# ucla-rlcourse/competitive-rl

Measured on AMD Instinct MI355X. Metric: env-steps/sec (whole node), cPongDouble 65536 envs per GPU, higher is better.
Workload: dtype u8; 1 GPU; cPongDouble-v0 raw (N,2,210,160,3) u8, 1 step = 1 frame (BASELINE config #2); envs_per_gpu=65536, gather=n/a, actions=uniform random, pre-generated on device, auto_reset=True

## Files before the change

### competitive_rl_amd/_native.py

```python
import ctypes as C
import os

import numpy as np

PKG = os.path.dirname(os.path.abspath(__file__))
LIB_PATH = os.path.join(PKG, "libcrl_hip_%s.so" % os.environ["CRL_LIB_VARIANT"] if os.environ.get("CRL_LIB_VARIANT") else "libcrl_hip.so")

CRL_ENV_PONG_DOUBLE, CRL_ENV_CAR_DOUBLE, CRL_ENV_PONG_SINGLE, CRL_ENV_CAR_SINGLE = 1, 2, 3, 4
CRL_FLAG_STACK_REPLICATE = 1
CAR_MAX_TILES = 512
CAR_MAP_ORG, CAR_MAP_W = 4392, 1216
CRL_OBS_RAW_RGB, CRL_OBS_GRAY_RESIZED = 0, 1
PONG_FRAME_BYTES = 210 * 160 * 3
ATLAS_BYTES = 22 * 22 * 34 * 160

CRL_LEAGUE_MAX_AGENTS = 16
CRL_LEAGUE_RANDOM, CRL_LEAGUE_RULE_BASED, CRL_LEAGUE_LIGHT = 0, 1, 2
CRL_POOL_KIND_FULL = 3
CRL_LEAGUE_DOMAIN_OPPONENT, CRL_LEAGUE_DOMAIN_ACTION, CRL_LEAGUE_DOMAIN_SAMPLE = 0x4C47554F, 0x4C475541, 0x4C475553
CRL_LEDGER_DOMAIN_OPPONENT = 0x4C475557
CRL_LEDGER_COUNTERS = 6
CRL_LEDGER_COUNTER_NAMES = ("episodes", "wins", "losses", "draws", "return_sum", "length_sum")
CRL_LEDGER_PFSP_HARD, CRL_LEDGER_PFSP_VARIANCE = 0, 1
CRL_ARENA_DOMAIN_PAIR = 0x4C475550
# ... 67 lines not shown
    "crl_car_get_track": (i32, [vp, i64, vp, vp, vp, vp, vp, vp]),
    "crl_car_set_track": (i32, [vp, i64, i32, vp, vp, vp, vp, vp]),
    "crl_car_get_map": (i32, [vp, i64, vp, vp, vp]),
    "crl_car_set_replay": (i32, [vp, vp, vp, i64]),
    "crl_policy_create": (i32, [i32, i64, vp, vp, vp, vp, vp, vp, P(vp)]),
    "crl_policy_create_full": (i32, [i32, i64, vp, vp, vp, vp, vp, vp, vp, vp, P(vp)]),
    "crl_policy_destroy": (None, [vp]),
    "crl_policy_reset": (i32, [vp, vp]),
    "crl_policy_act": (i32, [vp, vp, i64, vp, i64, vp, vp]),
    "crl_policy_get_stack": (i32, [vp, vp, vp]),
    "crl_policy_set_stack": (i32, [vp, vp, vp]),
    "crl_policy_set_sampling": (i32, [vp, f32, f32, u64, i64]),
    "crl_policy_set_critic": (i32, [vp, vp, vp]),
    "crl_policy_act_rollout": (i32, [vp, vp, i64, vp, vp, i64, vp, vp, vp, vp]),
    "crl_policy_load_weights": (i32, [vp, vp, vp, vp, vp, vp, vp, vp, vp, vp, vp, vp]),
    "crl_terminal_observation_dev": (i32, [vp, vp, i64, vp, vp]),
    "crl_check": (i32, [vp, vp]),
    "crl_car_info": (i32, [vp, P(vp), P(vp)]),
    "crl_car_copy_info": (i32, [vp, vp, vp, vp, vp]),
    "crl_frame_stack_update": (i32, [vp, vp, i32, i64, vp, i64, i32, i32, i64, vp]),
    "crl_frame_stack_update_to": (i32, [vp, vp, vp, i32, i64, vp, i64, i32, i32, i64, vp]),
    "crl_frame_stack_update_u8": (i32, [vp, vp, vp, i32, i64, vp, i64, i32, i32, i64, vp]),
    "crl_ctx_last_error": (cstr, [vp]),
    "crl_obs_descriptors": (i32, [vp, vp, vp]),
    "crl_render_frames_dev": (i32, [vp, vp, i64, vp, vp]),
    "crl_car_cap_hits": (i32, [vp, vp, vp]),
    "crl_selftest_sincosf": (i32, [i32, u64, u64, vp]),
    "crl_step_stack": (i32, [vp, vp, vp, vp, vp, P(CrlStackDesc), vp]),
    "crl_draw_stack": (i32, [vp, vp, P(CrlStackDesc), vp]),
    "crl_set_flags_event": (i32, [vp, vp]),
    "crl_kernel_time_stats": (i32, [vp, i32, P(f64), P(i64), P(f64)]),
    "crl_draw_raw_delta": (i32, [vp, vp, vp, i32, vp]),
    "crl_step_raw_delta": (i32, [vp, vp, vp, vp, vp, vp, vp]),
    "crl_league_create": (i32, [i32, i64, i64, u64, P(vp)]),
    "crl_league_destroy": (None, [vp]),
    "crl_league_add_builtin": (i32, [vp, i32]),
    "crl_league_add_light": (i32, [vp, vp, vp, vp, vp, vp, vp]),
    "crl_pool_add_full": (i32, [vp, vp, vp, vp, vp, vp, vp, vp, vp, i64]),
    "crl_pool_load_light": (i32, [vp, i32, vp, vp, vp, vp, vp, vp, vp]),
    "crl_pool_load_full": (i32, [vp, i32, vp, vp, vp, vp, vp, vp, vp, vp, vp]),
    "crl_sampling_set_agent": (i32, [vp, i32, f32, f32]),
    "crl_sampling_get_agent": (i32, [vp, i32, P(f32), P(f32)]),
    "crl_league_seed": (i32, [vp, u64, vp]),
    "crl_league_set_assignment": (i32, [vp, vp, i32, vp]),
    "crl_league_get_assignment": (i32, [vp, vp, vp]),
    "crl_league_resample": (i32, [vp, vp, vp]),
    "crl_league_get_lists": (i32, [vp, vp, vp, vp]),
    "crl_league_act": (i32, [vp, vp, i64, vp, i64, vp, vp]),
    "crl_league_reset": (i32, [vp, vp]),
    "crl_league_get_stack": (i32, [vp, vp, vp]),
    "crl_league_set_stack": (i32, [vp, vp, vp]),
    "crl_ledger_create": (i32, [i32, i64, i64, u64, i32, P(vp)]),
    "crl_ledger_destroy": (None, [vp]),
    "crl_ledger_seed": (i32, [vp, u64, vp]),
    "crl_ledger_reset": (i32, [vp, vp]),
    "crl_ledger_set_agents": (i32, [vp, i32, vp]),
    "crl_ledger_set_weights": (i32, [vp, vp, i32, vp]),
    "crl_ledger_get_weights": (i32, [vp, vp, vp]),
    "crl_ledger_pfsp_weights": (i32, [vp, vp, i32, i32, u32, vp]),
    "crl_ledger_get_counters": (i32, [vp, vp, vp, vp]),
    "crl_ledger_set_counters": (i32, [vp, vp, vp, vp]),
    "crl_ledger_get_env_state": (i32, [vp, vp, vp, vp, vp]),
    "crl_ledger_set_env_state": (i32, [vp, vp, vp, vp, vp]),
    "crl_ledger_step": (i32, [vp, vp, vp, i64, vp, i32, vp, vp]),
    "crl_arena_create": (i32, [i32, i64, i64, u64, i32, P(vp)]),
    "crl_arena_destroy": (None, [vp]),
# ... 71 lines not shown
```

### competitive_rl_amd/csrc/crl_api.hip

```cpp
#include <math.h>
#include <stdarg.h>
#include <stdio.h>
#include <string.h>

#include <algorithm>
#include <string>
#include <vector>

#include "crl_internal.h"
#include "pong_band_span.h"
#include "pong_device.h"

using namespace crl;

static thread_local std::string g_err;
static thread_local std::string *g_ctx_err = nullptr;

void crl_fail_no_ctx(void) { g_ctx_err = nullptr; }

int crl_fail(int code, const char *fmt, ...) {
    char buf[512];
    va_list ap;
    va_start(ap, fmt);
    vsnprintf(buf, sizeof(buf), fmt, ap);
// ... 7 lines not shown
    std::vector<int32_t> ofs, si;
    std::vector<float> alpha;
};

static AreaTab area_table(int ssize, int dsize) {
    AreaTab t;
    const double scale = 1.0 / ((double)dsize / (double)ssize);
    for (int d = 0; d < dsize; d++) {
        t.ofs.push_back((int32_t)t.si.size());
        const double f1 = d * scale, f2 = f1 + scale;
        const double cell = std::min(scale, ssize - f1);
        int s1 = (int)ceil(f1), s2 = (int)floor(f2);
        s2 = std::min(s2, ssize - 1);
        s1 = std::min(s1, s2);
        if (s1 - f1 > 1e-3) t.si.push_back(s1 - 1), t.alpha.push_back((float)((s1 - f1) / cell));
        for (int s = s1; s < s2; s++) t.si.push_back(s), t.alpha.push_back((float)(1.0 / cell));
        if (f2 - s2 > 1e-3) t.si.push_back(s2), t.alpha.push_back((float)(std::min(std::min(f2 - s2, 1.0), cell) / cell));
    }
    t.ofs.push_back((int32_t)t.si.size());
    return t;
}


struct crl_ctx {
    std::string err;
    crl_opts o;
    int64_t n;
    PongSoA s{};
    ServeSrc src{};
    std::vector<void *> allocs;
    uint8_t *atlas_rgb = nullptr;
    uint8_t *band_span = nullptr;
    int ink_row0 = 0, ink_row1 = 0;
    GrayTables gray{};
    uint8_t *tile_hdr = nullptr;
    double *ru = nullptr;
    uint8_t *rbx = nullptr, *rby = nullptr;
    crl_timer tm;
    uint64_t *gather = nullptr;
    int64_t gather_cap = 0;
    int64_t *idx_dev = nullptr;
    int64_t idx_cap = 0;
    int32_t *bad_action_host = nullptr, *bad_action_dev = nullptr;
    std::vector<uint8_t> atlas_host;
    hipEvent_t flags_ev = nullptr;
    crl_car_ctx *car = nullptr;
};

template <class T>
static int dev_alloc(crl_ctx *c, T **p, size_t count) {
    void *q = nullptr;
    HIP_TRY(hipMalloc(&q, std::max<size_t>(count * sizeof(T), 16)));
    c->allocs.push_back(q);
    *p = (T *)q;
    return CRL_OK;
}

template <class T>
static int dev_upload(crl_ctx *c, T **p, const std::vector<T> &v, size_t pad_to = 0) {
    size_t cnt = std::max(v.size(), pad_to);
    int rc = dev_alloc(c, p, cnt);
    if (rc) return rc;
    HIP_TRY(hipMemset(*p, 0, std::max<size_t>(cnt * sizeof(T), 16)));
    HIP_TRY(hipMemcpy(*p, v.data(), v.size() * sizeof(T), hipMemcpyHostToDevice));
    return CRL_OK;
}
// ... 231 lines not shown
        if (e == hipSuccess) e = hipMemset(c->s.num_steps, 0, n * 4);
        if (e == hipSuccess) e = hipMemset(c->s.real_reward, 0, n * 8);
        if (e == hipSuccess) e = hipMemcpy(c->s.keep, blank.data(), 2 * n * 8, hipMemcpyHostToDevice);
        if (e == hipSuccess) e = hipMemcpy(c->s.ring, blank.data(), 8 * n * 8, hipMemcpyHostToDevice);
        if (e == hipSuccess) e = hipMemcpy(c->s.obs_frames, blank.data(), 2 * n * 8, hipMemcpyHostToDevice);
        if (e == hipSuccess) e = hipMemcpy(c->s.term_frames, blank.data(), 2 * n * 8, hipMemcpyHostToDevice);
        if (e == hipSuccess) e = hipHostMalloc((void **)&c->bad_action_host, 64, hipHostMallocMapped);
        if (e == hipSuccess) {
            *c->bad_action_host = 0;
            e = hipHostGetDevicePointer((void **)&c->bad_action_dev, c->bad_action_host, 0);
        }
        if (e != hipSuccess) {
            crl_destroy(c);
            return crl_fail(CRL_EHIP, "create: state initialisation: %s", hipGetErrorString(e));
        }
        c->s.bad_action = c->bad_action_dev;
    }
    c->src.seed = opts->seed, c->src.env_id_base = opts->env_id_base;
    int r0 = CRL_PONG_TOP, r1 = 0;
    for (int sp = 0; sp < 484; sp++)
        for (int r = 0; r < CRL_PONG_TOP; r++)
            for (int x = 0; x < CRL_PONG_W; x++)
                if (c->atlas_host[((size_t)sp * CRL_PONG_TOP + r) * CRL_PONG_W + x] != 255) r0 = std::min(r0, r), r1 = std::max(r1, r + 1);
    if (r1 <= r0) r0 = r1 = 0;
    c->ink_row0 = r0, c->ink_row1 = r1;
    if (opts->obs_mode == CRL_OBS_RAW_RGB) {
        std::vector<uint8_t> rgb((size_t)CRL_PONG_ATLAS_BYTES * 3);
        for (size_t i = 0; i < (size_t)CRL_PONG_ATLAS_BYTES; i++) rgb[3 * i] = rgb[3 * i + 1] = rgb[3 * i + 2] = c->atlas_host[i];
        rc = dev_upload(c, &c->atlas_rgb, rgb);
        std::vector<uint8_t> span(pong_band_span_bytes(22));
        const int bad = pong_band_span_table(c->atlas_host.data(), 22, CRL_PONG_TOP, CRL_PONG_W, r0, r1, span.data());
        if (!rc && bad) rc = crl_fail(CRL_ESTATE, "score atlas: transition %d changes a pixel outside the ink rows [%d, %d)", bad - 1, r0, r1);
        if (!rc) rc = dev_upload(c, &c->band_span, span);
    } else {
        rc = setup_gray(c);
    }
    if (rc) { crl_destroy(c); return rc; }
    hipError_t e = hipDeviceSynchronize();
    if (e != hipSuccess) { crl_destroy(c); return crl_fail(CRL_EHIP, "create: %s", hipGetErrorString(e)); }
    *out = c;
    return CRL_OK;
}

void crl_destroy(crl_ctx *c) {
    g_ctx_err = nullptr;
    if (!c) return;
    hipSetDevice(c->o.device);
    hipDeviceSynchronize();
#ifdef CRL_ABLATION
    if (getenv("CRL_GRAY_DEBUG") && (atoi(getenv("CRL_GRAY_DEBUG")) & 128)) pong_gray_print_ticks();
#endif
    if (c->car) crl_car_destroy(c->car);
    for (void *p : c->allocs) hipFree(p);
    for (int w = 0; w < kTimerSlots; w++)
        for (auto &p : c->tm.ev[w]) hipEventDestroy(p.a), hipEventDestroy(p.b);
    for (auto &p : c->tm.pool) hipEventDestroy(p.a), hipEventDestroy(p.b);
    if (c->ru) hipFree(c->ru);
    if (c->rbx) hipFree(c->rbx);
    if (c->rby) hipFree(c->rby);
    if (c->gather) hipFree(c->gather);
    if (c->idx_dev) hipFree(c->idx_dev);
    if (c->bad_action_host) hipHostFree(c->bad_action_host);
    delete c;
}

int crl_seed(crl_ctx *c, uint64_t seed) {
// ... 129 lines not shown
    }
    end_timed(c, 1, st);
    HIP_TRY(hipGetLastError());
    return CRL_OK;
}

int crl_step_raw_delta(crl_ctx *c, const void *actions_void, uint8_t *obs_dev, uint64_t *drawn_dev, float *rew_dev, uint8_t *done_dev, void *stream) {
    CRL_ENTER(c);
    if (!c || !actions_void || !obs_dev || !drawn_dev) return crl_fail(CRL_EINVAL, "null argument");
    if (c->car || c->o.obs_mode != CRL_OBS_RAW_RGB) return crl_fail(CRL_ESTATE, "crl_step_raw_delta needs a Pong RAW_RGB context");
    if ((uintptr_t)obs_dev % 16) return crl_fail(CRL_EINVAL, "crl_step_raw_delta: obs_dev must be 16-byte aligned");
    if ((uintptr_t)drawn_dev % 8) return crl_fail(CRL_EINVAL, "crl_step_raw_delta: drawn_dev must be 8-byte aligned");
    if (int rc = pending_action_error(c, true)) return rc;
    hipStream_t st = (hipStream_t)stream;
    if (c->flags_ev) {
        begin_timed(c, 0, st);
        launch_pong_dynamics(c->s, c->src, (const int32_t *)actions_void, c->n, pong_mode(c), rew_dev, done_dev, st);
        end_timed(c, 0, st);
        HIP_TRY(hipGetLastError());
        HIP_TRY(hipEventRecord(c->flags_ev, st));
        begin_timed(c, 1, st);
        launch_pong_raster_raw_delta(c->s.obs_frames, drawn_dev, c->n, c->atlas_rgb, c->band_span, c->ink_row0, c->ink_row1, obs_dev, pong_views(c), st);
        end_timed(c, 1, st);
        HIP_TRY(hipGetLastError());
        return CRL_OK;
    }
#ifdef CRL_ABLATION
    if (getenv("CRL_RAW_STEP_SPLIT") && atoi(getenv("CRL_RAW_STEP_SPLIT"))) {
        begin_timed(c, 0, st);
        launch_pong_dynamics(c->s, c->src, (const int32_t *)actions_void, c->n, pong_mode(c), rew_dev, done_dev, st);
        end_timed(c, 0, st);
        begin_timed(c, 1, st);
        launch_pong_step_raw_delta(c->s, c->src, (const int32_t *)actions_void, c->n, rew_dev, done_dev, drawn_dev, c->atlas_rgb, c->band_span,
                                   c->ink_row0, c->ink_row1, obs_dev, pong_views(c), st, 1);
        end_timed(c, 1, st);
        HIP_TRY(hipGetLastError());
        return CRL_OK;
    }
#endif
    begin_timed(c, 1, st);
    launch_pong_step_raw_delta(c->s, c->src, (const int32_t *)actions_void, c->n, rew_dev, done_dev, drawn_dev, c->atlas_rgb, c->band_span, c->ink_row0,
                               c->ink_row1, obs_dev, pong_views(c), st);
    end_timed(c, 1, st);
    HIP_TRY(hipGetLastError());
    return CRL_OK;
}

int crl_set_flags_event(crl_ctx *c, void *event) {
    CRL_ENTER(c);
    if (!c) return crl_fail(CRL_EINVAL, "null ctx");
    if (c->car) return crl_fail(CRL_ESTATE, "crl_set_flags_event is a Pong entry point");
    c->flags_ev = (hipEvent_t)event;
    return CRL_OK;
}

int crl_draw_stack(crl_ctx *c, uint8_t *obs_dev, const crl_stack_desc *stack, void *stream) {
    CRL_ENTER(c);
    if (!c || !stack) return crl_fail(CRL_EINVAL, "null argument");
    GrayStack sk;
    if (int rc = stack_of(c, stack, &sk)) return rc;
    return draw_obs(c, obs_dev, (hipStream_t)stream, &sk);
}

int crl_info(crl_ctx *c, const float **real_reward_dev, const int32_t **num_steps_dev) {
    CRL_ENTER(c);
    if (!c) return crl_fail(CRL_EINVAL, "null ctx");
    if (c->car) return crl_fail(CRL_ESTATE, "crl_info is a Pong entry point");
    if (real_reward_dev) *real_reward_dev = c->s.real_reward;
    if (num_steps_dev) *num_steps_dev = c->s.num_steps;
    return CRL_OK;
}

int crl_copy_info(crl_ctx *c, float *rr_out, int32_t *ns_out, void *stream) {
    CRL_ENTER(c);
    if (!c) return crl_fail(CRL_EINVAL, "null ctx");
    if (c->car) return crl_fail(CRL_ESTATE, "crl_copy_info is a Pong entry point");
    hipStream_t st = (hipStream_t)stream;
// ... 325 lines not shown
```

### competitive_rl_amd/csrc/pong_device.h

```cpp
#pragma once
#include <hip/hip_runtime.h>
#include <stdint.h>

#include "../../include/crl.h"

namespace crl {

struct PongSoA {
    double *speed_x, *speed_y;
    int32_t *ball_x, *ball_y, *bat_l, *bat_r, *score_l, *score_r, *rounds, *steps, *wrap_steps;
    uint32_t *serve_ctr;
    uint64_t *keep;
    uint64_t *ring;
    uint64_t *obs_frames;
    uint64_t *term_frames;
    float *real_reward;
    int32_t *num_steps;
    int32_t *bad_action;
};

struct ServeSrc {
    uint64_t seed;
    int64_t env_id_base;
    const double *ru;
// ... 172 lines not shown
    if (!action_ok(a.x) || !action_ok(a.y)) *s.bad_action = (action_ok(a.x) ? a.y : a.x) + 1;
    int r_l, r_r;
    const bool done = frame_step(e, a.x, a.y, src, i, r_l, r_r);
    const float fl = (float)r_l, fr = (float)r_r;
    if (rew) {
        if (single) rew[i] = fl;
        else reinterpret_cast<float2 *>(rew)[i] = make_float2(fl, fr);
    }
    reinterpret_cast<float2 *>(s.real_reward)[i] = make_float2(fl, fr);
    if (done) {
        const uint64_t t = frame_of(e);
        s.term_frames[i] = t, s.term_frames[n + i] = t;
        game_reset(e, src, i);
    }
    if (done_out) done_out[i] = done ? 1 : 0;
    const uint64_t f = frame_of(e);
    s.obs_frames[i] = f;
    store_env(s, i, e);
    return f;
}

struct PongMode {
    bool wrapped, single, replicate;
};
void launch_pong_reset(const PongSoA &s, const ServeSrc &src, int64_t n, PongMode mode, hipStream_t st);
void launch_pong_dynamics(const PongSoA &s, const ServeSrc &src, const int32_t *actions, int64_t n, PongMode mode,
                          float *rew, uint8_t *done, hipStream_t st);
void launch_pong_gather_frames(const uint64_t *frames, const int64_t *idx_dev, int64_t count, int64_t n, uint64_t *ring_out,
                               hipStream_t st);
void launch_pong_raster_raw(const uint64_t *frames, int64_t n, const uint8_t *atlas_rgb, int ink_row0, int ink_row1,
                            uint8_t *obs, int views, hipStream_t st);
void launch_pong_raster_raw_delta(const uint64_t *frames, uint64_t *drawn, int64_t n, const uint8_t *atlas_rgb, const uint8_t *band_span,
                                  int ink_row0, int ink_row1, uint8_t *obs, int views, hipStream_t st);
void launch_pong_step_raw_delta(const PongSoA &s, const ServeSrc &src, const int32_t *actions, int64_t n, float *rew, uint8_t *done,
                                uint64_t *drawn, const uint8_t *atlas_rgb, const uint8_t *band_span, int ink_row0, int ink_row1, uint8_t *obs,
                                int views, hipStream_t st, int stepped = 0);

struct GrayTabOfs {
    int xa, ya, xs0, xn, ys0, yn, xf, xl, yf, yl, total, fast_ok, max_taps;
    int xa255, rowstatic, colstatic;
    int box32;
};
struct GrayStack {
    uint8_t *out;
    int k, view;
    int f32;
    int valid;
    int alias;
};
struct GrayTables {
    int R;
    uint8_t *atlas_gray;
    uint8_t *band;
    int band_rows, band_chunks;
    int32_t *xofs, *yofs;
    int32_t *xsi, *ysi;
    float *xalpha, *yalpha;
    uint8_t *rest;
    int zero_row0, zero_row1;
    uint8_t *x_first, *x_last;
    uint8_t *y_first, *y_last;
    uint8_t *tab_blob;
    GrayTabOfs tofs;
    float *f32_top;
    float *f32_bot;
    int f32_bot0;
    int f32_xtaps, f32_ytaps;
    int f32_map_row0, f32_map_rows;
};
// ... 16 lines not shown
```

### competitive_rl_amd/csrc/pong_raster_raw.hip

```cpp
#include <stdlib.h>

#include "crl_internal.h"
#include "pong_band_span.h"
#include "pong_device.h"

namespace crl {

static constexpr int kRowBytes = CRL_PONG_W * 3;
static constexpr int kRowChunks = kRowBytes / 16;
static constexpr int kFrameChunks = CRL_PONG_H * kRowChunks;

__device__ inline uint32_t nibble_to_bytes(uint32_t nib) {
    return ((nib * 0x00204081u) & 0x01010101u) * 0xFFu;
}

__device__ inline uint32_t span_bits(int a, int b) {
    a = max(a, 0), b = min(b, 16);
    return a < b ? (((1u << b) - 1u) & ~((1u << a) - 1u)) : 0u;
}

__device__ inline uint32_t bswap32(uint32_t v) { return __builtin_bswap32(v); }

__device__ __forceinline__ uint4 raw_chunk(const Frame &f, int q, const uint4 *__restrict__ atlas_rgb, int ink_row0, int ink_row1, int dbg) {
    const bool blank = f.sl == 255;
    const uint32_t bg = blank ? 0u : 0xFFFFFFFFu;
    const int view = q >= kFrameChunks;
    const int c = q - view * kFrameChunks;
    const int row = c / kRowChunks;
    const int cc = c - row * kRowChunks;
    const bool mirror = view && row >= CRL_PONG_MIRROR_ROW;
    const int sc = mirror ? (kRowChunks - 1 - cc) : cc;
    uint4 v = make_uint4(bg, bg, bg, bg);
    if (!blank && !(dbg & 1)) {
// ... 78 lines not shown

#endif

template <int ITERS, int VIEWS>
__global__ __launch_bounds__(256) void pong_raster_raw_sweep_kernel(const uint64_t *__restrict__ frames, const uint4 *__restrict__ atlas_rgb,
                                                                    int ink_row0, int ink_row1, uint4 *__restrict__ obs, int64_t n, int dbg) {
    constexpr int per_env = VIEWS * kFrameChunks;
    const int64_t total = n * per_env;
    const int64_t stride = (int64_t)gridDim.x * 256;
    Frame f0[ITERS], f1[ITERS];
    int q0[ITERS];
#pragma unroll
    for (int i = 0; i < ITERS; i++) {
        int64_t g0 = (int64_t)blockIdx.x * 256 + i * stride;
        g0 = g0 < total ? g0 : total - 1;
        const int64_t e0 = g0 / per_env;
        const int64_t e1 = e0 + 1 < n ? e0 + 1 : e0;
        f0[i] = unpack_frame(frames[e0]), f1[i] = unpack_frame(frames[e1]);
        q0[i] = (int)(g0 - e0 * per_env);
    }
#pragma unroll
    for (int i = 0; i < ITERS; i++) {
        const int64_t g = (int64_t)blockIdx.x * 256 + i * stride + threadIdx.x;
        if (g >= total) break;
        int q = q0[i] + (int)threadIdx.x;
        const bool second = q >= per_env;
        q -= second ? per_env : 0;
        obs[g] = raw_chunk(pick_frame(f0[i], f1[i], second), q, atlas_rgb, ink_row0, ink_row1, dbg);
    }
}

static constexpr int kDeltaL = 32, kDeltaG = 4;
static_assert(kFrameChunks % kDeltaG == 0, "a view starts on a block boundary");
static constexpr int kStepW = 1, kStepB = 16;
static constexpr bool kDeltaNT = false, kStepNT = true;

typedef uint32_t crl_u32x4 __attribute__((ext_vector_type(4)));
template <bool NT>
__device__ __forceinline__ void chunk_store(uint4 *p, const uint4 &v) {
    if (NT) __builtin_nontemporal_store(crl_u32x4{v.x, v.y, v.z, v.w}, reinterpret_cast<crl_u32x4 *>(p));
    else *p = v;
}

template <bool WRAP, bool NT>
__device__ __forceinline__ void court_store(uint4 *__restrict__ out, int q_view, const Frame &f, bool mirror, int row, int q_row, int q) {
    int o = q - q_row;
    if (WRAP) {
        const int w = (o >= kRowChunks) - (o < 0);
        row += w, o -= w * kRowChunks;
    }
    chunk_store<NT>(reinterpret_cast<uint4 *>(reinterpret_cast<char *>(out) + (uint32_t)((q_view + q) * 16)), court_chunk(f, row, mirror ? kRowChunks - 1 - o : o, mirror));
}

struct BallCols {
    int c0, c1;
    bool ok;
};
__device__ __forceinline__ BallCols ball_cols(int x) {
    const int b0 = max(3 * x, 0), b1 = min(3 * x + kBallBytes, kRowBytes);
    BallCols c;
    c.ok = b0 < b1, c.c0 = b0 >> 4, c.c1 = (max(b1, 1) - 1) >> 4;
    return c;
}

template <int G, bool NT>
__device__ __forceinline__ void raw_delta_draw(uint64_t pn, uint64_t po, int view, int lane, uint4 *__restrict__ out, const uint4 *__restrict__ atlas_rgb,
                                               const uint8_t *__restrict__ band_span, int ink_row0, int ink_row1) {
    static_assert(G == 1 || G == 4, "");
// ... 94 lines not shown
    constexpr int E = 64 / L / VIEWS;
    static_assert((VIEWS == 1 || VIEWS == 2) && B <= 64 && B % W == 0 && B / W <= 16 && W % E == 0 && (W & (W - 1)) == 0, "");
    const int wave = __builtin_amdgcn_readfirstlane((int)threadIdx.x >> 6), wl = (int)threadIdx.x & 63;
    const int64_t b0 = (int64_t)blockIdx.x * B, e0 = b0 + wave * W;
    __shared__ uint64_t hand[2][B];
    if (wave == 0 && wl < B) {
        uint64_t pn = kBlankFrame, po = kBlankFrame;
        const int64_t i = b0 + wl;
        if (i < n) {
            po = drawn[i];
            pn = stepped ? s.obs_frames[i] : raw_step_env(s, src, actions, i, n, rew, done_out, VIEWS == 1);
            drawn[i] = pn;
        }
        hand[0][wl] = pn, hand[1][wl] = po;
    }
    __syncthreads();
    const int k = wave * W + (wl & (W - 1));
    const uint64_t pn = wl < W ? hand[0][k] : kBlankFrame, po = wl < W ? hand[1][k] : kBlankFrame;
    const int lane = wl & (L - 1), sub = wl / L;
#pragma unroll 1
    for (int t = 0; t < W; t += E) {
        if (e0 + t >= n) break;
        uint32_t nl, nh, ol, oh;
        if (VIEWS == 2) {
            nl = __builtin_amdgcn_readlane((uint32_t)pn, t), nh = __builtin_amdgcn_readlane((uint32_t)(pn >> 32), t);
            ol = __builtin_amdgcn_readlane((uint32_t)po, t), oh = __builtin_amdgcn_readlane((uint32_t)(po >> 32), t);
        } else {
            nl = __shfl((uint32_t)pn, t + sub), nh = __shfl((uint32_t)(pn >> 32), t + sub);
            ol = __shfl((uint32_t)po, t + sub), oh = __shfl((uint32_t)(po >> 32), t + sub);
        }
        const int64_t env = e0 + t + (VIEWS == 1 ? sub : 0);
        raw_delta_draw<G, NT>(((uint64_t)nh << 32) | nl, ((uint64_t)oh << 32) | ol, VIEWS == 2 ? sub : 0, lane, obs + env * per_env, atlas_rgb, band_span,
                              ink_row0, ink_row1);
    }
}

#ifdef CRL_ABLATION
static constexpr int kBatLc0 = 3 * CRL_PONG_BATL_X / 16, kBatLc1 = (3 * (CRL_PONG_BATL_X + CRL_PONG_BAT_W) - 1) / 16;
static constexpr int kBatRc0 = 3 * CRL_PONG_BATR_X / 16, kBatRc1 = (3 * (CRL_PONG_BATR_X + CRL_PONG_BAT_W) - 1) / 16;

struct DeltaRect {
    int r0, nr, o0, o1;
};

__device__ __forceinline__ DeltaRect delta_rect(int view, int r0, int r1, int c0, int c1) {
    r0 = max(r0, CRL_PONG_TOP), r1 = min(r1, CRL_PONG_BOTTOM);
    const bool mirror = view != 0;
    DeltaRect r;
    r.r0 = r0, r.nr = max(r1 - r0, 0);
    r.o0 = mirror ? kRowChunks - 1 - c1 : c0, r.o1 = mirror ? kRowChunks - 1 - c0 : c1;
    return r;
}

__device__ __forceinline__ void delta_bat(DeltaRect *r, int view, int a, int b, int c0, int c1) {
    const int lo = min(a, b), hi = max(a, b), k = min(hi - lo, CRL_PONG_BAT_H);
    r[0] = delta_rect(view, lo, lo + k, c0, c1);
    r[1] = delta_rect(view, hi + CRL_PONG_BAT_H - k, hi + CRL_PONG_BAT_H, c0, c1);
}

__device__ __forceinline__ DeltaRect delta_ball(int view, const Frame &g, bool moved) {
    const int b0 = max(3 * g.x, 0), b1 = min(3 * (g.x + CRL_PONG_BALL), kRowBytes);
    DeltaRect r = delta_rect(view, g.y, g.y + CRL_PONG_BALL, b0 / 16, (max(b1, 1) - 1) / 16);
    if (!moved || b0 >= b1) r.nr = 0;
    return r;
}

// ... 159 lines not shown
        else CRL_LAUNCH_DELTA((pong_raster_raw_delta_slots_kernel<1, L, G>), 1, L);               \
        return;                                                                                   \
    }
        CRL_DELTA_CASE(16, 1) CRL_DELTA_CASE(16, 2) CRL_DELTA_CASE(16, 4) CRL_DELTA_CASE(32, 1) CRL_DELTA_CASE(32, 2) CRL_DELTA_CASE(32, 4)
        CRL_DELTA_CASE(64, 1) CRL_DELTA_CASE(64, 2) CRL_DELTA_CASE(64, 4)
#undef CRL_DELTA_CASE
        return;
    }
#endif
    const bool blocks_ok = (uintptr_t)obs % (16 * kDeltaG) == 0;
    static const bool band_whole = CRL_ABL(getenv("CRL_RAW_BAND_WHOLE") && atoi(getenv("CRL_RAW_BAND_WHOLE")));
    const uint8_t *span = band_whole ? nullptr : band_span;
#define CRL_LAUNCH_DELTA_SPAN(V, G, NT)                                                                                                    \
    hipLaunchKernelGGL((pong_raster_raw_delta_kernel<V, G, NT>), dim3((unsigned)((n * V * kDeltaL + 255) / 256)), dim3(256), 0, st, frames, drawn, at, \
                       span, ink_row0, ink_row1, ob, n)
#ifdef CRL_ABLATION
    const bool abl_nt = getenv("CRL_RAW_NT") && atoi(getenv("CRL_RAW_NT"));
    if (abl_nt != kDeltaNT && views == 2 && blocks_ok) {
        CRL_LAUNCH_DELTA_SPAN(2, kDeltaG, !kDeltaNT);
        return;
    }
#endif
    if (views == 2) {
        if (blocks_ok) CRL_LAUNCH_DELTA_SPAN(2, kDeltaG, kDeltaNT);
        else CRL_LAUNCH_DELTA_SPAN(2, 1, kDeltaNT);
    } else {
        if (blocks_ok) CRL_LAUNCH_DELTA_SPAN(1, kDeltaG, kDeltaNT);
        else CRL_LAUNCH_DELTA_SPAN(1, 1, kDeltaNT);
    }
#undef CRL_LAUNCH_DELTA_SPAN
#undef CRL_LAUNCH_DELTA
}

void launch_pong_step_raw_delta(const PongSoA &s, const ServeSrc &src, const int32_t *actions, int64_t n, float *rew, uint8_t *done,
                                uint64_t *drawn, const uint8_t *atlas_rgb, const uint8_t *band_span, int ink_row0, int ink_row1, uint8_t *obs,
                                int views, hipStream_t st, int stepped) {
    if (n <= 0 || (views != 1 && views != 2)) return;
    const uint4 *at = reinterpret_cast<const uint4 *>(atlas_rgb);
    uint4 *ob = reinterpret_cast<uint4 *>(obs);
    const bool blocks_ok = (uintptr_t)obs % (16 * kDeltaG) == 0;
#define CRL_LAUNCH_STEP(V, G, W, B, NT)                                                                                                          \
    hipLaunchKernelGGL((pong_step_raw_delta_kernel<V, G, W, B, NT>), dim3((unsigned)((n + B - 1) / B)), dim3(64 * (B / W)), 0, st, s, src, actions, n, rew, \
                       done, drawn, at, band_span, ink_row0, ink_row1, ob, stepped)
#ifdef CRL_ABLATION
    const int abl_w = getenv("CRL_RAW_STEP_W") ? atoi(getenv("CRL_RAW_STEP_W")) : kStepW;
    const int abl_b = getenv("CRL_RAW_STEP_B") ? atoi(getenv("CRL_RAW_STEP_B")) : kStepB;
    const int abl_nt = getenv("CRL_RAW_NT") ? atoi(getenv("CRL_RAW_NT")) : (int)kStepNT;
    if (views == 2 && blocks_ok && (abl_w != kStepW || abl_b != kStepB || (abl_nt != 0) != kStepNT)) {
#define CRL_STEP_CASE(W, B)                                            \
    if (abl_w == W && abl_b == B) {                                    \
        if (abl_nt) CRL_LAUNCH_STEP(2, kDeltaG, W, B, true);           \
        else CRL_LAUNCH_STEP(2, kDeltaG, W, B, false);                 \
        return;                                                        \
    }
        CRL_STEP_CASE(1, 16) CRL_STEP_CASE(2, 16) CRL_STEP_CASE(2, 32) CRL_STEP_CASE(4, 32) CRL_STEP_CASE(4, 64) CRL_STEP_CASE(8, 64) CRL_STEP_CASE(16, 64)
        CRL_STEP_CASE(32, 64) CRL_STEP_CASE(64, 64) CRL_STEP_CASE(1, 8) CRL_STEP_CASE(1, 4)
#undef CRL_STEP_CASE
        return;
    }
#endif
    constexpr int W1 = kStepW < 2 ? 2 : kStepW;
    if (views == 2) {
        if (blocks_ok) CRL_LAUNCH_STEP(2, kDeltaG, kStepW, kStepB, kStepNT);
        else CRL_LAUNCH_STEP(2, 1, kStepW, kStepB, kStepNT);
    } else {
        if (blocks_ok) CRL_LAUNCH_STEP(1, kDeltaG, W1, kStepB, kStepNT);
        else CRL_LAUNCH_STEP(1, 1, W1, kStepB, kStepNT);
    }
#undef CRL_LAUNCH_STEP
}

void launch_pong_raster_raw(const uint64_t *frames, int64_t n, const uint8_t *atlas_rgb, int ink_row0, int ink_row1,
                            uint8_t *obs, int views, hipStream_t st) {
    if (n <= 0) return;
    static const int dbg = CRL_ABL(getenv("CRL_RAW_DEBUG") ? atoi(getenv("CRL_RAW_DEBUG")) : 0);
    static const int sweep = CRL_ABL(getenv("CRL_RAW_SWEEP") != nullptr) ? atoi(getenv("CRL_RAW_SWEEP")) : 4;
    if (views != 1 && views != 2) return;
    if (sweep > 0) {
        const int64_t total = n * views * kFrameChunks;
        const uint4 *at = reinterpret_cast<const uint4 *>(atlas_rgb);
        uint4 *ob = reinterpret_cast<uint4 *>(obs);
#define CRL_LAUNCH_SWEEP(I, V)                                                                                              \
    hipLaunchKernelGGL((pong_raster_raw_sweep_kernel<I, V>), dim3((unsigned)((total + 256 * I - 1) / (256 * I))), dim3(256), 0, st, frames, \
                       at, ink_row0, ink_row1, ob, n, dbg)
        if (views == 2) {
#ifdef CRL_ABLATION
            if (sweep <= 2) CRL_LAUNCH_SWEEP(2, 2);
            else if (sweep > 4) CRL_LAUNCH_SWEEP(8, 2);
            else
#endif
                CRL_LAUNCH_SWEEP(4, 2);
        } else {
            CRL_LAUNCH_SWEEP(4, 1);
        }
#undef CRL_LAUNCH_SWEEP
        return;
    }
#ifdef CRL_ABLATION
    static const int lin = getenv("CRL_RAW_LINEAR") ? atoi(getenv("CRL_RAW_LINEAR")) : 2;
    if (lin > 0) {
        const int64_t total = n * views * kFrameChunks;
// ... 23 lines not shown
```

### competitive_rl_amd/vec_env.py

```python
import ctypes as C
from abc import ABC, abstractmethod

import numpy as np
import torch

from . import _native as N
from . import spaces

CHEAT_CODES = 999


class VecEnv(ABC):

    metadata = {"render.modes": ["human", "rgb_array"]}

    def __init__(self, num_envs, observation_space, action_space):
        self.num_envs = num_envs
        self.observation_space = observation_space
        self.action_space = action_space

    @abstractmethod
    def reset(self):
        pass

# ... 582 lines not shown
        N.check(self._L.crl_render_raw(self._h, frames.ctypes.data_as(C.c_void_p), len(frames),
                                       C.c_void_p(out.data_ptr()), self._stream()))
        return out

    def obs_descriptors(self, out=None):
        if out is None:
            out = torch.empty((8, self.num_envs), dtype=torch.int64, device=self.device)
        assert out.is_contiguous() and out.numel() == 8 * self.num_envs and out.element_size() == 8 and out.device == self.device
        N.check(self._L.crl_obs_descriptors(self._h, C.c_void_p(out.data_ptr()), self._stream()))
        return out

    def render_descriptors(self, desc, out=None):
        assert desc.is_contiguous() and desc.element_size() == 8 and desc.device == self.device and desc.numel() % 8 == 0
        count = desc.numel() // 8
        if out is None:
            out = torch.empty((count,) + tuple(self._obs_shape[1:]), dtype=self._buf_dtype, device=self.device)
        assert out.is_contiguous() and out.device == self.device
        N.check(self._L.crl_render_frames_dev(self._h, C.c_void_p(desc.data_ptr()), count, C.c_void_p(out.data_ptr()), self._stream()))
        return out

    def step_device(self, actions_i32, render=True, obs_out=None):
        if not (actions_i32.is_contiguous() and actions_i32.dtype == torch.int32 and actions_i32.device == self.device):
            raise AssertionError("step_device needs a contiguous int32 tensor on the env's device")
        if obs_out is not None:
            if not (obs_out.is_contiguous() and obs_out.dtype == self._buf_dtype and obs_out.device == self.device
                    and obs_out.numel() == self._obs[0].numel()):
                raise AssertionError("obs_out must be a contiguous tensor of the observation buffer's size and dtype on the env's device")
        buf, _ = self._step(actions_i32, alias_ok=False, render=render or obs_out is not None, obs_out=obs_out)
        return buf, self._rew, self._done

    def kernel_timing(self, enable=True):
        N.check(self._L.crl_kernel_timing(self._h, int(enable)))

    def kernel_time_ms(self, which):
        ms, cnt = C.c_double(), C.c_int64()
        N.check(self._L.crl_kernel_time_ms(self._h, which, C.byref(ms), C.byref(cnt)))
        return ms.value, cnt.value

    def kernel_time_stats(self, which):
        ms, cnt, mx = C.c_double(), C.c_int64(), C.c_double()
        N.check(self._L.crl_kernel_time_stats(self._h, which, C.byref(ms), C.byref(cnt), C.byref(mx)))
        return ms.value, cnt.value, mx.value


class _EnvList:
    def __init__(self, venv):
        self._venv = venv

    def __len__(self):
        return self._venv.num_envs

    def __getitem__(self, i):
        if not -len(self) <= i < len(self):
            raise IndexError(i)
        return _EnvHandle(self._venv, i % len(self))

    def __iter__(self):
        return (self[i] for i in range(len(self)))
```

### include/crl.h

```cpp
#ifndef CRL_H_
#define CRL_H_

#include <stdint.h>

#ifdef __cplusplus
extern "C" {
#endif

#define CRL_PONG_W 160
#define CRL_PONG_H 210
#define CRL_PONG_TOP 34
#define CRL_PONG_BOTTOM 194
#define CRL_PONG_BALL 4
#define CRL_PONG_BAT_W 5
#define CRL_PONG_BAT_H 15
#define CRL_PONG_BATL_X 16
#define CRL_PONG_BATR_X 139
#define CRL_PONG_MIRROR_ROW 25
#define CRL_PONG_MAX_ROUNDS 21
#define CRL_PONG_MAX_STEPS 10000
#define CRL_PONG_CHEAT 999
#define CRL_PONG_FRAME_BYTES (CRL_PONG_H * CRL_PONG_W * 3)
#define CRL_PONG_ATLAS_SCORES 22
#define CRL_PONG_ATLAS_BYTES (22 * 22 * CRL_PONG_TOP * CRL_PONG_W)
// ... 68 lines not shown
    CRL_OBS_F32_REF = 2,
};

typedef struct crl_ctx crl_ctx;

int crl_create(const crl_opts *opts, const uint8_t *score_atlas_host, crl_ctx **out);

void crl_destroy(crl_ctx *ctx);

int crl_seed(crl_ctx *ctx, uint64_t seed);

int crl_reset(crl_ctx *ctx, uint8_t *obs_dev, void *stream);

int crl_step(crl_ctx *ctx, const void *actions_dev, uint8_t *obs_dev, float *rew_dev,
             uint8_t *done_dev, void *stream);

typedef struct crl_stack_desc {
    void *stack_dev;
    int32_t planes;
    int32_t dtype;
    int32_t agent;
    int32_t valid_planes;
    int32_t alias_newest;
    int32_t reserved;
} crl_stack_desc;
int crl_step_stack(crl_ctx *ctx, const void *actions_dev, uint8_t *obs_dev, float *rew_dev, uint8_t *done_dev,
                   const crl_stack_desc *stack, void *stream);
int crl_draw_stack(crl_ctx *ctx, uint8_t *obs_dev, const crl_stack_desc *stack, void *stream);

int crl_draw_raw_delta(crl_ctx *ctx, uint8_t *obs_dev, uint64_t *drawn_dev, int32_t drawn_valid, void *stream);

int crl_step_raw_delta(crl_ctx *ctx, const void *actions_dev, uint8_t *obs_dev, uint64_t *drawn_dev, float *rew_dev, uint8_t *done_dev,
                       void *stream);

int crl_set_flags_event(crl_ctx *ctx, void *event);

int crl_info(crl_ctx *ctx, const float **real_reward_dev, const int32_t **num_steps_dev);
int crl_copy_info(crl_ctx *ctx, float *real_reward_out_dev, int32_t *num_steps_out_dev, void *stream);

int crl_terminal_observation(crl_ctx *ctx, const int64_t *env_idx_host, int64_t count,
                             uint8_t *out_dev, void *stream);

int crl_terminal_observation_dev(crl_ctx *ctx, const int64_t *env_idx_dev, int64_t count,
                                 uint8_t *out_dev, void *stream);

int crl_check(crl_ctx *ctx, void *stream);

int crl_get_state(crl_ctx *ctx, crl_pong_env_state *state_host, int64_t first, int64_t count,
                  void *stream);
int crl_set_state(crl_ctx *ctx, const crl_pong_env_state *state_host, int64_t first,
                  int64_t count, void *stream);

int crl_set_replay(crl_ctx *ctx, const double *u_host, const uint8_t *bx_host,
                   const uint8_t *by_host, int64_t per_env);

int crl_render_raw(crl_ctx *ctx, const crl_pong_frame *frames_host, int64_t count,
                   uint8_t *out_dev, void *stream);

int crl_obs_descriptors(crl_ctx *ctx, crl_pong_frame *desc_out_dev, void *stream);
int crl_render_frames_dev(crl_ctx *ctx, const crl_pong_frame *desc_dev, int64_t count, uint8_t *out_dev, void *stream);

int crl_render(crl_ctx *ctx, uint8_t *obs_dev, void *stream);

int64_t crl_obs_bytes_per_env(const crl_ctx *ctx);

int crl_kernel_timing(crl_ctx *ctx, int enable);
// ... 189 lines not shown
```

Before: 787.8 million env-steps/s.

## Replace raw-delta step kernel with persistent producer/consumer pipelined kernel

Swaps the one-shot fused step+draw kernel for a persistent, occupancy-sized grid. In each block one wave steps the next chunk of envs into double-buffered shared memory while D draw waves rasterize the previous chunk, taking work through an LDS atomic ticket. The goal is to overlap the latency-bound physics step with the bandwidth-bound frame writes and to balance uneven draw work. It adds block-level syncs and makes one wave serialize stepping for each chunk, which could become the bottleneck. It also adds an API to cap the number of resident groups.

```diff
diff --git a/competitive_rl_amd/_native.py b/competitive_rl_amd/_native.py
--- a/competitive_rl_amd/_native.py
+++ b/competitive_rl_amd/_native.py
@@ -123,6 +123,7 @@
     "crl_kernel_time_stats": (i32, [vp, i32, P(f64), P(i64), P(f64)]),
     "crl_draw_raw_delta": (i32, [vp, vp, vp, i32, vp]),
     "crl_step_raw_delta": (i32, [vp, vp, vp, vp, vp, vp, vp]),
+    "crl_set_raw_step_groups": (i32, [vp, i32]),
     "crl_league_create": (i32, [i32, i64, i64, u64, P(vp)]),
     "crl_league_destroy": (None, [vp]),
     "crl_league_add_builtin": (i32, [vp, i32]),
diff --git a/competitive_rl_amd/csrc/crl_api.hip b/competitive_rl_amd/csrc/crl_api.hip
--- a/competitive_rl_amd/csrc/crl_api.hip
+++ b/competitive_rl_amd/csrc/crl_api.hip
@@ -63,6 +63,8 @@
     uint8_t *atlas_rgb = nullptr;
     uint8_t *band_span = nullptr;
     int ink_row0 = 0, ink_row1 = 0;
+    int raw_step_held[2] = {1, 1};
+    int raw_step_cap = 0;
     GrayTables gray{};
     uint8_t *tile_hdr = nullptr;
     double *ru = nullptr;
@@ -360,6 +362,7 @@
         const int bad = pong_band_span_table(c->atlas_host.data(), 22, CRL_PONG_TOP, CRL_PONG_W, r0, r1, span.data());
         if (!rc && bad) rc = crl_fail(CRL_ESTATE, "score atlas: transition %d changes a pixel outside the ink rows [%d, %d)", bad - 1, r0, r1);
         if (!rc) rc = dev_upload(c, &c->band_span, span);
+        pong_step_raw_delta_groups(pong_views(c), c->raw_step_held);
     } else {
         rc = setup_gray(c);
     }
@@ -555,7 +558,7 @@
         end_timed(c, 0, st);
         begin_timed(c, 1, st);
         launch_pong_step_raw_delta(c->s, c->src, (const int32_t *)actions_void, c->n, rew_dev, done_dev, drawn_dev, c->atlas_rgb, c->band_span,
-                                   c->ink_row0, c->ink_row1, obs_dev, pong_views(c), st, 1);
+                                   c->ink_row0, c->ink_row1, obs_dev, pong_views(c), st, c->raw_step_held, c->raw_step_cap, 1);
         end_timed(c, 1, st);
         HIP_TRY(hipGetLastError());
         return CRL_OK;
@@ -563,9 +566,18 @@
 #endif
     begin_timed(c, 1, st);
     launch_pong_step_raw_delta(c->s, c->src, (const int32_t *)actions_void, c->n, rew_dev, done_dev, drawn_dev, c->atlas_rgb, c->band_span, c->ink_row0,
-                               c->ink_row1, obs_dev, pong_views(c), st);
+                               c->ink_row1, obs_dev, pong_views(c), st, c->raw_step_held, c->raw_step_cap);
     end_timed(c, 1, st);
     HIP_TRY(hipGetLastError());
+    return CRL_OK;
+}
+
+int crl_set_raw_step_groups(crl_ctx *c, int32_t groups) {
+    CRL_ENTER(c);
+    if (!c) return crl_fail(CRL_EINVAL, "null ctx");
+    if (c->car || c->o.obs_mode != CRL_OBS_RAW_RGB) return crl_fail(CRL_ESTATE, "crl_set_raw_step_groups needs a Pong RAW_RGB context");
+    if (groups < 0) return crl_fail(CRL_EINVAL, "crl_set_raw_step_groups: groups must be >= 0 (0: as many as the device holds)");
+    c->raw_step_cap = groups;
     return CRL_OK;
 }
 
diff --git a/competitive_rl_amd/csrc/pong_device.h b/competitive_rl_amd/csrc/pong_device.h
--- a/competitive_rl_amd/csrc/pong_device.h
+++ b/competitive_rl_amd/csrc/pong_device.h
@@ -228,9 +228,10 @@
                             uint8_t *obs, int views, hipStream_t st);
 void launch_pong_raster_raw_delta(const uint64_t *frames, uint64_t *drawn, int64_t n, const uint8_t *atlas_rgb, const uint8_t *band_span,
                                   int ink_row0, int ink_row1, uint8_t *obs, int views, hipStream_t st);
+void pong_step_raw_delta_groups(int views, int groups[2]);
 void launch_pong_step_raw_delta(const PongSoA &s, const ServeSrc &src, const int32_t *actions, int64_t n, float *rew, uint8_t *done,
                                 uint64_t *drawn, const uint8_t *atlas_rgb, const uint8_t *band_span, int ink_row0, int ink_row1, uint8_t *obs,
-                                int views, hipStream_t st, int stepped = 0);
+                                int views, hipStream_t st, const int groups[2], int cap, int stepped = 0);
 
 struct GrayTabOfs {
     int xa, ya, xs0, xn, ys0, yn, xf, xl, yf, yl, total, fast_ok, max_taps;
diff --git a/competitive_rl_amd/csrc/pong_raster_raw.hip b/competitive_rl_amd/csrc/pong_raster_raw.hip
--- a/competitive_rl_amd/csrc/pong_raster_raw.hip
+++ b/competitive_rl_amd/csrc/pong_raster_raw.hip
@@ -1,4 +1,6 @@
 #include <stdlib.h>
+
+#include <algorithm>
 
 #include "crl_internal.h"
 #include "pong_band_span.h"
@@ -143,8 +145,11 @@
 
 static constexpr int kDeltaL = 32, kDeltaG = 4;
 static_assert(kFrameChunks % kDeltaG == 0, "a view starts on a block boundary");
-static constexpr int kStepW = 1, kStepB = 16;
-static constexpr bool kDeltaNT = false, kStepNT = true;
+[[maybe_unused]] static constexpr int kStepW = 1, kStepB = 16;
+static constexpr bool kDeltaNT = false;
+[[maybe_unused]] static constexpr bool kStepNT = true;
+static constexpr int kPipeD = 7, kPipeC = 64;
+static constexpr bool kPipeTicket = true, kPipeNT = false;
 
 typedef uint32_t crl_u32x4 __attribute__((ext_vector_type(4)));
 template <bool NT>
@@ -305,6 +310,67 @@
         const int64_t env = e0 + t + (VIEWS == 1 ? sub : 0);
         raw_delta_draw<G, NT>(((uint64_t)nh << 32) | nl, ((uint64_t)oh << 32) | ol, VIEWS == 2 ? sub : 0, lane, obs + env * per_env, atlas_rgb, band_span,
                               ink_row0, ink_row1);
+    }
+}
+
+template <int VIEWS, int G, int D, int C, bool TK, bool NT>
+__global__ __launch_bounds__(64 * (D + 1)) void pong_step_raw_pipe_kernel(
+    PongSoA s, ServeSrc src, const int32_t *__restrict__ actions, int64_t n, float *__restrict__ rew, uint8_t *__restrict__ done_out,
+    uint64_t *__restrict__ drawn, const uint4 *__restrict__ atlas_rgb, const uint8_t *__restrict__ band_span, int ink_row0, int ink_row1,
+    uint4 *__restrict__ obs, int stepped) {
+    constexpr int L = kDeltaL, per_env = VIEWS * kFrameChunks;
+    constexpr int E = 64 / L / VIEWS;
+    static_assert((VIEWS == 1 || VIEWS == 2) && D >= 1 && D <= 15 && C >= E && C <= 64 && C % E == 0, "");
+    const int wave = __builtin_amdgcn_readfirstlane((int)threadIdx.x >> 6), wl = (int)threadIdx.x & 63;
+    const int lane = wl & (L - 1), sub = wl / L;
+    const int64_t chunks = (n + C - 1) / C;
+    __shared__ uint64_t hand[2][2][C];
+    __shared__ int ticket[2];
+    int slot = 0;
+    if (wave == 0) {
+#pragma unroll 1
+        for (int64_t next = blockIdx.x, cur = -1; cur < chunks; cur = next, next += gridDim.x, slot ^= 1) {
+            if (next < chunks) {
+                if (wl < C) {
+                    uint64_t pn = kBlankFrame, po = kBlankFrame;
+                    const int64_t i = next * C + wl;
+                    if (i < n) {
+                        pn = stepped ? s.obs_frames[i] : raw_step_env(s, src, actions, i, n, rew, done_out, VIEWS == 1);
+                        po = drawn[i];
+                        drawn[i] = pn;
+                    }
+                    hand[slot][0][wl] = pn, hand[slot][1][wl] = po;
+                }
+                if (wl == 0) ticket[slot] = 0;
+            }
+            __syncthreads();
+        }
+        return;
+    }
+#pragma unroll 1
+    for (int64_t next = blockIdx.x, cur = -1; cur < chunks; cur = next, next += gridDim.x, slot ^= 1) {
+        if (cur >= 0) {
+            const int from = slot ^ 1;
+            const int64_t e0 = cur * C;
+            const int cnt = (int)min((int64_t)C, n - e0);
+#pragma unroll 1
+            for (int t = wave - 1;; t += D) {
+                if (TK) {
+                    int v = 0;
+                    if (wl == 0) v = atomicAdd(&ticket[from], 1);
+                    t = __builtin_amdgcn_readfirstlane(v);
+                }
+                if (t * E >= cnt) break;
+                const int e = t * E + (VIEWS == 1 ? sub : 0);
+                uint64_t pn = hand[from][0][e], po = hand[from][1][e];
+                if (VIEWS == 2) {
+                    pn = ((uint64_t)__builtin_amdgcn_readfirstlane((uint32_t)(pn >> 32)) << 32) | __builtin_amdgcn_readfirstlane((uint32_t)pn);
+                    po = ((uint64_t)__builtin_amdgcn_readfirstlane((uint32_t)(po >> 32)) << 32) | __builtin_amdgcn_readfirstlane((uint32_t)po);
+                }
+                raw_delta_draw<G, NT>(pn, po, VIEWS == 2 ? sub : 0, lane, obs + (e0 + e) * per_env, atlas_rgb, band_span, ink_row0, ink_row1);
+            }
+        }
+        __syncthreads();
     }
 }
 
@@ -530,9 +596,28 @@
 #undef CRL_LAUNCH_DELTA
 }
 
+template <int V, int G, int D, int C, bool TK, bool NT>
+static int pipe_groups() {
+    int dev = 0, cus = 0, per = 0;
+    if (hipGetDevice(&dev) != hipSuccess || hipDeviceGetAttribute(&cus, hipDeviceAttributeMultiprocessorCount, dev) != hipSuccess ||
+        hipOccupancyMaxActiveBlocksPerMultiprocessor(&per, pong_step_raw_pipe_kernel<V, G, D, C, TK, NT>, 64 * (D + 1), 0) != hipSuccess) {
+        (void)hipGetLastError();
+        return 1;
+    }
+    return std::max(1, per * cus);
+}
+
+void pong_step_raw_delta_groups(int views, int groups[2]) {
+    if (views == 2) {
+        groups[0] = pipe_groups<2, 1, kPipeD, kPipeC, kPipeTicket, kPipeNT>(), groups[1] = pipe_groups<2, kDeltaG, kPipeD, kPipeC, kPipeTicket, kPipeNT>();
+    } else {
+        groups[0] = pipe_groups<1, 1, kPipeD, kPipeC, kPipeTicket, kPipeNT>(), groups[1] = pipe_groups<1, kDeltaG, kPipeD, kPipeC, kPipeTicket, kPipeNT>();
+    }
+}
+
 void launch_pong_step_raw_delta(const PongSoA &s, const ServeSrc &src, const int32_t *actions, int64_t n, float *rew, uint8_t *done,
                                 uint64_t *drawn, const uint8_t *atlas_rgb, const uint8_t *band_span, int ink_row0, int ink_row1, uint8_t *obs,
-                                int views, hipStream_t st, int stepped) {
+                                int views, hipStream_t st, const int groups[2], int cap, int stepped) {
     if (n <= 0 || (views != 1 && views != 2)) return;
     const uint4 *at = reinterpret_cast<const uint4 *>(atlas_rgb);
     uint4 *ob = reinterpret_cast<uint4 *>(obs);
@@ -540,11 +625,16 @@
 #define CRL_LAUNCH_STEP(V, G, W, B, NT)                                                                                                          \
     hipLaunchKernelGGL((pong_step_raw_delta_kernel<V, G, W, B, NT>), dim3((unsigned)((n + B - 1) / B)), dim3(64 * (B / W)), 0, st, s, src, actions, n, rew, \
                        done, drawn, at, band_span, ink_row0, ink_row1, ob, stepped)
+#define CRL_LAUNCH_PIPE(V, G, D, C, TK, NT, held)                                                                                                \
+    hipLaunchKernelGGL((pong_step_raw_pipe_kernel<V, G, D, C, TK, NT>),                                                                          \
+                       dim3((unsigned)std::min<int64_t>((n + C - 1) / C, std::max(1, cap > 0 ? std::min(cap, (held)) : (held)))), dim3(64 * (D + 1)), 0, st, s, \
+                       src, actions, n, rew, done, drawn, at, band_span, ink_row0, ink_row1, ob, stepped)
 #ifdef CRL_ABLATION
+    const bool abl_old = getenv("CRL_RAW_STEP_W") || getenv("CRL_RAW_STEP_B");
     const int abl_w = getenv("CRL_RAW_STEP_W") ? atoi(getenv("CRL_RAW_STEP_W")) : kStepW;
     const int abl_b = getenv("CRL_RAW_STEP_B") ? atoi(getenv("CRL_RAW_STEP_B")) : kStepB;
-    const int abl_nt = getenv("CRL_RAW_NT") ? atoi(getenv("CRL_RAW_NT")) : (int)kStepNT;
-    if (views == 2 && blocks_ok && (abl_w != kStepW || abl_b != kStepB || (abl_nt != 0) != kStepNT)) {
+    const int abl_nt = getenv("CRL_RAW_NT") ? atoi(getenv("CRL_RAW_NT")) : (int)(abl_old ? kStepNT : kPipeNT);
+    if (views == 2 && blocks_ok && abl_old) {
 #define CRL_STEP_CASE(W, B)                                            \
     if (abl_w == W && abl_b == B) {                                    \
         if (abl_nt) CRL_LAUNCH_STEP(2, kDeltaG, W, B, true);           \
@@ -556,15 +646,39 @@
 #undef CRL_STEP_CASE
         return;
     }
+    const int abl_d = getenv("CRL_RAW_PIPE_D") ? atoi(getenv("CRL_RAW_PIPE_D")) : kPipeD;
+    const int abl_c = getenv("CRL_RAW_PIPE_C") ? atoi(getenv("CRL_RAW_PIPE_C")) : kPipeC;
+    const int abl_tk = getenv("CRL_RAW_PIPE_TICKET") ? atoi(getenv("CRL_RAW_PIPE_TICKET")) : (int)kPipeTicket;
+    if (views == 2 && blocks_ok && (abl_d != kPipeD || abl_c != kPipeC || (abl_tk != 0) != kPipeTicket || (abl_nt != 0) != kPipeNT)) {
+#define CRL_PIPE_CASE_(D, C, TK, NT)                                                \
+    {                                                                               \
+        static const int held = pipe_groups<2, kDeltaG, D, C, TK, NT>();            \
+        CRL_LAUNCH_PIPE(2, kDeltaG, D, C, TK, NT, held);                            \
+        return;                                                                     \
+    }
+#define CRL_PIPE_CASE(D, C)                                                         \
+    if (abl_d == D && abl_c == C) {                                                 \
+        if (abl_tk && abl_nt) CRL_PIPE_CASE_(D, C, true, true)                      \
+        if (abl_tk) CRL_PIPE_CASE_(D, C, true, false)                               \
+        if (abl_nt) CRL_PIPE_CASE_(D, C, false, true)                               \
+        CRL_PIPE_CASE_(D, C, false, false)                                          \
+    }
+        CRL_PIPE_CASE(4, 32) CRL_PIPE_CASE(7, 32) CRL_PIPE_CASE(15, 32) CRL_PIPE_CASE(4, 64) CRL_PIPE_CASE(7, 64) CRL_PIPE_CASE(15, 64)
+        CRL_PIPE_CASE(6, 64) CRL_PIPE_CASE(11, 64) CRL_PIPE_CASE(13, 64)
+#undef CRL_PIPE_CASE
+#undef CRL_PIPE_CASE_
+        return;
+    }
 #endif
-    constexpr int W1 = kStepW < 2 ? 2 : kStepW;
+    const int held = groups[blocks_ok ? 1 : 0];
     if (views == 2) {
-        if (blocks_ok) CRL_LAUNCH_STEP(2, kDeltaG, kStepW, kStepB, kStepNT);
-        else CRL_LAUNCH_STEP(2, 1, kStepW, kStepB, kStepNT);
+        if (blocks_ok) CRL_LAUNCH_PIPE(2, kDeltaG, kPipeD, kPipeC, kPipeTicket, kPipeNT, held);
+        else CRL_LAUNCH_PIPE(2, 1, kPipeD, kPipeC, kPipeTicket, kPipeNT, held);
     } else {
-        if (blocks_ok) CRL_LAUNCH_STEP(1, kDeltaG, W1, kStepB, kStepNT);
-        else CRL_LAUNCH_STEP(1, 1, W1, kStepB, kStepNT);
-    }
+        if (blocks_ok) CRL_LAUNCH_PIPE(1, kDeltaG, kPipeD, kPipeC, kPipeTicket, kPipeNT, held);
+        else CRL_LAUNCH_PIPE(1, 1, kPipeD, kPipeC, kPipeTicket, kPipeNT, held);
+    }
+#undef CRL_LAUNCH_PIPE
 #undef CRL_LAUNCH_STEP
 }
 
diff --git a/competitive_rl_amd/vec_env.py b/competitive_rl_amd/vec_env.py
--- a/competitive_rl_amd/vec_env.py
+++ b/competitive_rl_amd/vec_env.py
@@ -638,6 +638,9 @@
     def kernel_timing(self, enable=True):
         N.check(self._L.crl_kernel_timing(self._h, int(enable)))
 
+    def set_raw_step_groups(self, groups=0):
+        N.check(self._L.crl_set_raw_step_groups(self._h, int(groups)))
+
     def kernel_time_ms(self, which):
         ms, cnt = C.c_double(), C.c_int64()
         N.check(self._L.crl_kernel_time_ms(self._h, which, C.byref(ms), C.byref(cnt)))
diff --git a/include/crl.h b/include/crl.h
--- a/include/crl.h
+++ b/include/crl.h
@@ -124,6 +124,8 @@
 
 int crl_step_raw_delta(crl_ctx *ctx, const void *actions_dev, uint8_t *obs_dev, uint64_t *drawn_dev, float *rew_dev, uint8_t *done_dev,
                        void *stream);
+
+int crl_set_raw_step_groups(crl_ctx *ctx, int32_t groups);
 
 int crl_set_flags_event(crl_ctx *ctx, void *event);
 
```

Measured after the change: 769.0 million env-steps/s. 2.4% lower.
